# meuleman/epilogos

Hardware: AMD Instinct MI355X
Metric: Mbins scored/sec (S1, 18-state, 833 biosamples) (higher is better)
Workload: dtype u8

## Files before the change

### epilogos_amd/csrc/epg_s1.hip

```cpp
#include "epg_count.h"

#include <stdlib.h>
#include <string.h>

namespace epg {

typedef unsigned short k1_v2u16 __attribute__((ext_vector_type(2)));

constexpr int K1P_LD = 17;

template <int SC, bool FULL, bool PAIRS, typename Loop>
__device__ __forceinline__ void bin_hist_body(int Sout_, u64* __restrict__ counts, int nmax, u64* __restrict__ counts2, Loop&& loop) {
    constexpr int S = SC;
    constexpr int ND = (S + 1) / 2;
    const int Sout = FULL ? S : Sout_;
    const int ROWB = 2 * Sout;
    __shared__ u64 s_cnt[S + 1];
    __shared__ __attribute__((aligned(16))) char s_stage[4][32 * 2 * S];
    constexpr int PG = (S + 2) / 3, PSP = 3 * PG, PROLES = PG * (PG + 1) / 2, PSLICE = PROLES <= 64 ? 64 / PROLES : 1;
    static_assert(!PAIRS || (FULL && PROLES <= 64), "the pair counts need a compile-time row width and at most 64 block roles");
    __shared__ u32 s_pair[PAIRS ? 4 * PSP * K1P_LD : 1];
    __shared__ u64 s_c2[PAIRS ? S * S : 1];
    const int lane = threadIdx.x & 63, wave = threadIdx.x >> 6;
    const int j = lane & 3, b = lane >> 2;
    if (threadIdx.x <= S) s_cnt[threadIdx.x] = 0;
    if (PAIRS) {
        for (int e = threadIdx.x; e < S * S; e += 256) s_c2[e] = 0;
        for (int e = threadIdx.x; e < 4 * PSP * K1P_LD; e += 256) s_pair[e] = 0;
    }
    __syncthreads();
    u16* H = nullptr;
    int pgi = -1, pgj = 0, pkq = 0;
    u64 pacc[PAIRS ? 9 : 1], prs[PAIRS ? 3 : 1];
    if (PAIRS) {
        const int role = lane < PROLES * PSLICE ? lane / PSLICE : -1;
        pkq = lane % PSLICE;
        if (role >= 0) {
            int t = role, i = 0;
            while (t >= PG - i) { t -= PG - i; ++i; }
            pgi = i; pgj = i + t;
        }
#pragma unroll
        for (int c = 0; c < 9; ++c) pacc[c] = 0;
#pragma unroll
        for (int c = 0; c < 3; ++c) prs[c] = 0;
    }
    auto pair_counts = [&](const char* stage, int rows) {
        u32* sp = s_pair + wave * PSP * K1P_LD;
        const u16* raw = reinterpret_cast<const u16*>(stage);
        __builtin_amdgcn_wave_barrier();
        for (int e = lane; e < S * 16; e += 64) {
            const int i = e >> 4, k = e & 15;
            const u32 lo = 2 * k < rows ? raw[(2 * k) * S + i] : 0u, hi = 2 * k + 1 < rows ? raw[(2 * k + 1) * S + i] : 0u;
            sp[i * K1P_LD + k] = lo | (hi << 16);
        }
        __builtin_amdgcn_wave_barrier();
        if (pgi >= 0) {
            const u32* pi = sp + 3 * pgi * K1P_LD;
            const u32* pj = sp + 3 * pgj * K1P_LD;
            u32 part[9] = {0, 0, 0, 0, 0, 0, 0, 0, 0}, ps[3] = {0, 0, 0};
            const bool diag = pgi == pgj;
            for (int k = pkq; k < 16; k += PSLICE) {
                const u32 av[3] = {pi[k], pi[K1P_LD + k], pi[2 * K1P_LD + k]};
                const u32 bv[3] = {pj[k], pj[K1P_LD + k], pj[2 * K1P_LD + k]};
#pragma unroll
                for (int t = 0; t < 3; ++t)
#pragma unroll
                    for (int u = 0; u < 3; ++u)
                        part[3 * t + u] = __builtin_amdgcn_udot2(__builtin_bit_cast(k1_v2u16, av[t]), __builtin_bit_cast(k1_v2u16, bv[u]), part[3 * t + u], false);
                if (diag) {
#pragma unroll
                    for (int t = 0; t < 3; ++t)
                        ps[t] = __builtin_amdgcn_udot2(__builtin_bit_cast(k1_v2u16, av[t]), __builtin_bit_cast(k1_v2u16, 0x00010001u), ps[t], false);
                }
            }
#pragma unroll
            for (int c = 0; c < 9; ++c) pacc[c] += part[c];
#pragma unroll
            for (int c = 0; c < 3; ++c) prs[c] += ps[c];
        }
        __builtin_amdgcn_wave_barrier();
    };

    u32 accp[ND];
#pragma unroll
    for (int m = 0; m < ND; ++m) accp[m] = 0;
    const int flush_every = 65535 / nmax > 1 ? 65535 / nmax - 1 : 1;
    int since = 0;
    auto flush = [&]() {
        if (j == 0) {
#pragma unroll
            for (int m = 0; m < ND; ++m) {
                const u32 lo = accp[m] & 0xffffu, hi = accp[m] >> 16;
                if (lo) atomicAdd(&s_cnt[2 * m], (u64)lo);
                if (hi) atomicAdd(&s_cnt[2 * m + 1], (u64)hi);
            }
        }
#pragma unroll
        for (int m = 0; m < ND; ++m) accp[m] = 0;
        since = 0;
    };

    auto enter = [&](u16* Hpart) { H = Hpart; };
    auto epilogue = [&](int half, long row, bool valid, u32 (&cnt)[S]) {
        u32 d[ND];
        pack_reduce<S>(cnt, d);
        if (counts) {
#pragma unroll
            for (int m = 0; m < ND; ++m) accp[m] += valid ? d[m] : 0u;
            if (++since >= flush_every) flush();
        }
        if (H) {
            char* srow = &s_stage[wave][(half * 16 + b) * ROWB];
            if constexpr (FULL && (S & 1) == 0) {
#pragma unroll
                for (int k = 0; k < (ND + 3) / 4; ++k) {
                    const u32 v = sel4(d[4 * k], 4 * k + 1 < ND ? d[4 * k + 1] : 0u, 4 * k + 2 < ND ? d[4 * k + 2] : 0u,
                                       4 * k + 3 < ND ? d[4 * k + 3] : 0u, j);
                    if (4 * k + j < ND) *reinterpret_cast<u32*>(srow + 4 * (4 * k + j)) = v;
                }
            } else {
#pragma unroll
                for (int k = 0; k < (S + 3) / 4; ++k) {
                    const u32 v = (j & 2) ? (2 * k + 1 < ND ? d[2 * k + 1] : 0u) : d[2 * k];
                    const u32 c = (j & 1) ? v >> 16 : v & 0xffffu;
                    if (4 * k + j < Sout) *reinterpret_cast<u16*>(srow + 2 * (4 * k + j)) = (u16)c;
                }
            }
        }
    };
    auto finish = [&](long st, long row0, int rows) {
        if (H) store_staged(s_stage[wave], reinterpret_cast<char*>(H) + row0 * ROWB, rows * ROWB, lane);
        if constexpr (PAIRS) pair_counts(s_stage[wave], rows);
    };
    loop(enter, epilogue, finish);

    if (counts) {
        flush();
        __syncthreads();
        if ((int)threadIdx.x < Sout && s_cnt[threadIdx.x]) atomicAdd(&counts[threadIdx.x], s_cnt[threadIdx.x]);
    }
    if constexpr (PAIRS) {
        if (pgi >= 0) {
            const bool diag = pgi == pgj;
#pragma unroll
            for (int t = 0; t < 3; ++t)
#pragma unroll
                for (int u = 0; u < 3; ++u) {
                    const int i = 3 * pgi + t, jj = 3 * pgj + u;
                    u64 v = pacc[3 * t + u];
                    if (diag && t == u) v -= prs[t];
                    if (i >= S || jj >= S || !v) continue;
                    atomicAdd(&s_c2[i * S + jj], v);
                    if (!diag) atomicAdd(&s_c2[jj * S + i], v);
                }
        }
        __syncthreads();
        for (int e = threadIdx.x; e < S * S; e += 256)
            if (s_c2[e]) atomicAdd(&counts2[e], s_c2[e]);
    }
}

template <int SC, int NG, bool FULL>
__global__ __launch_bounds__(256) void k_bin_hist(const char* __restrict__ X, long R, int N, long ldx, int Sout_,
                                                   u16* __restrict__ H, u64* __restrict__ counts) {
    bin_hist_body<SC, FULL, false>(Sout_, counts, N, nullptr, [&](auto&& enter, auto&& epilogue, auto&& finish) {
        enter(H);
        tile_loop<SC, NG>(X, R, N, ldx, epilogue, finish);
    });
}

template <int SC, int NG>
__global__ __launch_bounds__(256) void k_bin_hist_s2(const char* __restrict__ X, long R, int N, long ldx, u16* __restrict__ H,
                                                      u64* __restrict__ counts, u64* __restrict__ counts2) {
    bin_hist_body<SC, true, true>(SC, counts, N, counts2, [&](auto&& enter, auto&& epilogue, auto&& finish) {
        enter(H);
        tile_loop<SC, NG>(X, R, N, ldx, epilogue, finish);
    });
}

template <int SC, int NG, bool FULL>
__global__ __launch_bounds__(256) void k_bin_hist_parts(const KhParts pt, int Sout_, u64* __restrict__ counts, int nmax) {
    bin_hist_body<SC, FULL, false>(Sout_, counts, nmax, nullptr, [&](auto&& enter, auto&& epilogue, auto&& finish) {
        tile_loop_parts<SC, NG>(pt, [&](int part) { enter(pt.h[part]); }, epilogue, finish);
    });
}

__global__ __launch_bounds__(256) void k_bin_hist_safe(const char* __restrict__ X, long row_begin, long row_end, int N,
                                                        long ldx, int S, u16* __restrict__ H, u64* __restrict__ counts, int mask = 31) {
    __shared__ u32 s_h[4][128];
    const int lane = threadIdx.x & 63, wave = threadIdx.x >> 6;
    for (long row = row_begin + (long)blockIdx.x * 4 + wave; row < row_end; row += (long)gridDim.x * 4) {
        for (int s = lane; s < S; s += 64) s_h[wave][s] = 0;
        __builtin_amdgcn_wave_barrier();
        const char* rp = X + row * ldx;
        for (int n = lane; n < N; n += 64) {
            const int v = (unsigned char)rp[n] & mask;
            if (v < S) atomicAdd(&s_h[wave][v], 1u);
        }
        __builtin_amdgcn_wave_barrier();
        for (int s = lane; s < S; s += 64) {
            const u32 c = s_h[wave][s];
            if (H) H[row * S + s] = (u16)c;
            if (counts && c) atomicAdd(&counts[s], (u64)c);
        }
        __builtin_amdgcn_wave_barrier();
    }
}

__global__ void k_s1_table(const float* __restrict__ q, int N, int S, double* __restrict__ T64, float* __restrict__ T32) {
    const long e = (long)blockIdx.x * blockDim.x + threadIdx.x;
    if (e >= (long)(N + 1) * S) return;
    const int c = (int)(e / S), s = (int)(e % S);
    const double p = (double)c / (double)N;
    const double v = kl_term(p, (double)q[s]);
    T64[e] = v;
    T32[e] = (float)v;
}

template <int S, int NG, typename OT>
__global__ __launch_bounds__(256) void k_score_s1(const char* __restrict__ X, long R, int N, long ldx,
                                                   const OT* __restrict__ T, OT* __restrict__ out) {
    constexpr int ND = (S + 1) / 2;
    constexpr int ROWB = S * (int)sizeof(OT);
    __shared__ __attribute__((aligned(16))) char s_stage[4][32 * ROWB];
    const int lane = threadIdx.x & 63, wave = threadIdx.x >> 6;
    const int j = lane & 3, b = lane >> 2;
    auto epilogue = [&](int half, long row, bool valid, u32 (&cnt)[S]) {
        u32 d[ND];
        pack_reduce<S>(cnt, d);
        OT* srow = reinterpret_cast<OT*>(&s_stage[wave][(half * 16 + b) * ROWB]);
#pragma unroll
        for (int k = 0; k < (S + 3) / 4; ++k) {
            const u32 v = (j & 2) ? (2 * k + 1 < ND ? d[2 * k + 1] : 0u) : d[2 * k];
            const u32 c = (j & 1) ? v >> 16 : v & 0xffffu;
            const int s = 4 * k + j;
            if (s < S) srow[s] = (c && valid) ? T[(long)c * S + s] : (OT)0;
        }
    };
    auto finish = [&](long st, long row0, int rows) {
        store_staged_nt(s_stage[wave], reinterpret_cast<char*>(out) + row0 * ROWB, rows * ROWB, lane);
    };
    tile_loop<S, NG>(X, R, N, ldx, epilogue, finish);
}

template <typename OT, bool LDS_T>
__global__ __launch_bounds__(LDS_T ? 1024 : 256) void k_score_s1_from_hist(const u16* __restrict__ H, long total, int S,
                                                                             const OT* __restrict__ Tg, int nent, OT* __restrict__ out,
                                                                             u64* __restrict__ zero_counts, int rev) {
    extern __shared__ __attribute__((aligned(16))) char smem_t[];
    if (zero_counts && blockIdx.x == 0 && (int)threadIdx.x < S) zero_counts[threadIdx.x] = 0;
    const OT* T = Tg;
    if (LDS_T) {
        OT* Ts = reinterpret_cast<OT*>(smem_t);
        for (int e = threadIdx.x; e < nent; e += blockDim.x) Ts[e] = Tg[e];
        __syncthreads();
        T = Ts;
    }
    const u32 cmax = (u32)(nent / S - 1);
    const long nquads = total >> 2;
    const long stride = (long)gridDim.x * blockDim.x;
    long qd = (long)blockIdx.x * blockDim.x + threadIdx.x;
    const long qtop = nquads - 1, qsgn = rev ? -1 : 1, qoff = rev ? qtop : 0;
    for (; qd + 3 * stride < nquads; qd += 4 * stride) {
        uint2 h[4];
#pragma unroll
        for (int u = 0; u < 4; ++u) h[u] = *reinterpret_cast<const uint2*>(H + 4 * (qoff + qsgn * (qd + u * stride)));
#pragma unroll
        for (int u = 0; u < 4; ++u) {
            const long e0 = 4 * (qoff + qsgn * (qd + u * stride));
            int s = (int)(e0 % S);
            const u32 c[4] = {h[u].x & 0xffffu, h[u].x >> 16, h[u].y & 0xffffu, h[u].y >> 16};
            OT v[4];
#pragma unroll
            for (int k = 0; k < 4; ++k) {
                v[k] = c[k] - 1u < cmax ? T[(long)c[k] * S + s] : (OT)0;
                s = s + 1 == S ? 0 : s + 1;
            }
            if constexpr (sizeof(OT) == 4) {
                typedef float v4f_nt __attribute__((ext_vector_type(4)));
                const v4f_nt vv = {(float)v[0], (float)v[1], (float)v[2], (float)v[3]};
                __builtin_nontemporal_store(vv, reinterpret_cast<v4f_nt*>(out + e0));
            } else {
                typedef double v2d_nt __attribute__((ext_vector_type(2)));
                const v2d_nt lo = {(double)v[0], (double)v[1]}, hi = {(double)v[2], (double)v[3]};
                __builtin_nontemporal_store(lo, reinterpret_cast<v2d_nt*>(out + e0));
                __builtin_nontemporal_store(hi, reinterpret_cast<v2d_nt*>(out + e0 + 2));
            }
        }
    }
    for (; qd < nquads; qd += stride) {
        const long e0 = 4 * (qoff + qsgn * qd);
        int s = (int)(e0 % S);
        for (int k = 0; k < 4; ++k) {
            const u32 c = H[e0 + k];
            out[e0 + k] = c - 1u < cmax ? T[(long)c * S + s] : (OT)0;
            s = s + 1 == S ? 0 : s + 1;
        }
    }
    if (blockIdx.x == 0 && threadIdx.x < (total & 3)) {
        const long e = (nquads << 2) + threadIdx.x;
        const u32 c = H[e];
        out[e] = c - 1u < cmax ? T[(long)c * S + (int)(e % S)] : (OT)0;
    }
}

template <typename IT>
__global__ __launch_bounds__(256) void k_sum_int(const IT* __restrict__ C, long n, long long* __restrict__ total) {
    long long acc = 0;
    for (long i = (long)blockIdx.x * blockDim.x + threadIdx.x; i < n; i += (long)gridDim.x * blockDim.x) acc += (long long)C[i];
    for (int off = 32; off > 0; off >>= 1) acc += __shfl_down(acc, off);
    __shared__ long long s_part[4];
    if ((threadIdx.x & 63) == 0) s_part[threadIdx.x >> 6] = acc;
    __syncthreads();
    if (threadIdx.x == 0) {
        const long long t = s_part[0] + s_part[1] + s_part[2] + s_part[3];
        if (t) atomicAdd(reinterpret_cast<u64*>(total), (u64)t);
    }
}

template <typename IT>
__global__ __launch_bounds__(256) void k_normalise(const IT* __restrict__ C, long n, const long long* __restrict__ total,
                                                    float* __restrict__ q) {
    const double tot = (double)(*total);
    for (long i = (long)blockIdx.x * blockDim.x + threadIdx.x; i < n; i += (long)gridDim.x * blockDim.x)
        q[i] = (float)((double)C[i] / tot);
}

template <typename IT>
__global__ __launch_bounds__(256) void k_normalise_small(const IT* __restrict__ C, int n, float* __restrict__ q) {
    __shared__ long long s_part[4];
    long long acc = 0;
    for (int i = threadIdx.x; i < n; i += 256) acc += (long long)C[i];
    for (int off = 32; off > 0; off >>= 1) acc += __shfl_down(acc, off);
    if ((threadIdx.x & 63) == 0) s_part[threadIdx.x >> 6] = acc;
    __syncthreads();
    const double tot = (double)(s_part[0] + s_part[1] + s_part[2] + s_part[3]);
    for (int i = threadIdx.x; i < n; i += 256) q[i] = (float)((double)C[i] / tot);
}

static int blocks_per_cu() { return g_force[FORCE_K1_BLOCKS_PER_CU] > 0 ? g_force[FORCE_K1_BLOCKS_PER_CU] : 2; }
static int grid_for_tiles(long R) {
    const long nsuper = (R + 31) >> 5;
    long blocks = (nsuper + 3) / 4;
    const long cap = (long)num_cus() * blocks_per_cu();
    if (blocks > cap) {
        const long iters = (nsuper + cap * 4 - 1) / (cap * 4);
        blocks = (nsuper + iters * 4 - 1) / (iters * 4);
    }
    if (blocks < 1) blocks = 1;
    return (int)blocks;
}

template <typename F>
static void with_count_core(int S, int ng, F&& f) {
    if (S == 15 || S == 18 || S == 25)
        with_constant<25, 15, 18>(S, [&](auto sc) {
            with_constant<0, 1, 2, 3, 4, 5, 6, 7, 8>(ng, [&](auto NG) { f(sc, NG, std::true_type{}); });
        });
    else
        with_constant<31, 15, 18, 25>(S < 15 ? 15 : S < 18 ? 18 : S < 25 ? 25 : 31,
                                      [&](auto sc) { f(sc, std::integral_constant<int, 0>{}, std::false_type{}); });
}

static long fast_rows(long R, int N, long ldx) {
    const long chunks = (N + 15) / 16;
    const long over = 16 * chunks - ldx;
    if (over <= 0) return R;
    const long unsafe = (over + ldx - 1) / ldx;
    return R > unsafe ? R - unsafe : 0;
}

extern "C" int epg_bin_hist(const int8_t* X8, int64_t R, int32_t N, int64_t ldx, int32_t S, uint16_t* H, int64_t* counts, void* stream) {
    hipStream_t st = (hipStream_t)stream;
    if (R < 0 || N < 1 || ldx < N || S < 1) return fail(EPG_ERR_INVALID_ARG, "bin_hist: bad shape R=%lld N=%d ldx=%lld S=%d", (long long)R, N, (long long)ldx, S);
    if (S > 127) return fail(EPG_ERR_UNSUPPORTED, "bin_hist: S=%d > 127 (states are int8)", S);
    if (N > 65535) return fail(EPG_ERR_UNSUPPORTED, "bin_hist: N=%d > 65535 (uint16 per-bin counts)", N);
    if (R == 0) return EPG_OK;
    if (!X8) return fail(EPG_ERR_INVALID_ARG, "bin_hist: X is NULL");
    if (H && (reinterpret_cast<uintptr_t>(H) & 15)) return fail(EPG_ERR_INVALID_ARG, "bin_hist: H must be 16-byte aligned");
    const char* X = reinterpret_cast<const char*>(X8);
    u64* cnt = reinterpret_cast<u64*>(counts);
    if (S > 31) {
        hipLaunchKernelGGL(k_bin_hist_safe, dim3((unsigned)((R + 3) / 4 < num_cus() * 32L ? (R + 3) / 4 : num_cus() * 32L)), dim3(256), 0, st, X, 0L,
                           (long)R, N, ldx, S, H, cnt, 255);
        EPG_LAUNCH_CHECK("k_bin_hist_safe");
        return EPG_OK;
    }
    const long Rf = fast_rows(R, N, ldx);
    if (Rf > 0) {
        with_count_core(S, (N + 127) / 128, [&](auto SC, auto NG, auto MODEL) {
            hipLaunchKernelGGL((k_bin_hist<SC, NG, MODEL && (SC & 1) == 0>), dim3(grid_for_tiles(Rf)), dim3(256), 0, st, X, Rf, N, ldx, S, H, cnt);
        });
        EPG_LAUNCH_CHECK("k_bin_hist");
    }
    if (Rf < R) {
        hipLaunchKernelGGL(k_bin_hist_safe, dim3((unsigned)((R - Rf + 3) / 4 < 1024 ? (R - Rf + 3) / 4 : 1024)), dim3(256), 0, st, X, Rf, (long)R, N, ldx, S, H, cnt);
        EPG_LAUNCH_CHECK("k_bin_hist_safe");
    }
    return EPG_OK;
}

extern "C" int epg_bin_hist_s2(const int8_t* X8, int64_t R, int32_t N, int64_t ldx, int32_t S, uint16_t* H, int64_t* counts, int64_t* counts2,
                               void* stream) {
    hipStream_t st = (hipStream_t)stream;
    if (!H || !counts2) return fail(EPG_ERR_INVALID_ARG, "bin_hist_s2: H and counts2 are required");
    const bool fused = (S == 15 || S == 18 || S == 25) && R > 0 && N >= 1 && N <= 1024 && ldx >= N && X8 &&
                       !(reinterpret_cast<uintptr_t>(H) & 15) && fast_rows(R, N, ldx) == R;
    if (!fused) {
        int rc = epg_bin_hist(X8, R, N, ldx, S, H, counts, stream);
        if (rc) return rc;
        return epg_hist_s2_from_binhist(H, R, S, counts2, stream);
    }
    const char* X = reinterpret_cast<const char*>(X8);
    u64* c1 = reinterpret_cast<u64*>(counts);
    u64* c2 = reinterpret_cast<u64*>(counts2);
    with_constant<25, 18, 15>(S, [&](auto SC) {
        with_constant<8, 1, 2, 3, 4, 5, 6, 7>((N + 127) / 128, [&](auto NG) {
            hipLaunchKernelGGL((k_bin_hist_s2<decltype(SC)::value, NG>), dim3(grid_for_tiles(R)), dim3(256), 0, st, X, R, N, ldx, H, c1, c2);
        });
    });
    EPG_LAUNCH_CHECK("k_bin_hist_s2");
    return EPG_OK;
}

extern "C" int epg_bin_hist_parts(int32_t nparts, const int8_t* const* X, const int64_t* R, const int32_t* N, const int64_t* ldx, int32_t S,
                                  uint16_t* const* H, int64_t* counts, void* stream) {
    hipStream_t st = (hipStream_t)stream;
    if (nparts < 0 || (nparts && (!X || !R || !N || !ldx))) return fail(EPG_ERR_INVALID_ARG, "bin_hist_parts: NULL argument array");
    if (S < 1 || S > 127) return fail(EPG_ERR_UNSUPPORTED, "bin_hist_parts: S=%d outside 1..127", S);
    for (int p = 0; p < nparts; ++p) {
        if (R[p] < 0 || (R[p] && (N[p] < 1 || ldx[p] < N[p]))) return fail(EPG_ERR_INVALID_ARG, "bin_hist_parts: bad shape of part %d", p);
        if (R[p] && N[p] > 65535) return fail(EPG_ERR_UNSUPPORTED, "bin_hist_parts: N=%d > 65535 (uint16 per-bin counts)", N[p]);
        if (R[p] && !X[p]) return fail(EPG_ERR_INVALID_ARG, "bin_hist_parts: X of part %d is NULL", p);
        if (H && H[p] && (reinterpret_cast<uintptr_t>(H[p]) & 15)) return fail(EPG_ERR_INVALID_ARG, "bin_hist_parts: H of part %d must be 16-byte aligned", p);
    }
    if (S > 31) {
        for (int p = 0; p < nparts; ++p) {
            const int rc = epg_bin_hist(X[p], R[p], N[p], ldx[p], S, H ? H[p] : nullptr, counts, stream);
            if (rc) return rc;
        }
        return EPG_OK;
    }
    u64* cnt = reinterpret_cast<u64*>(counts);
    auto cls = [](int n) { const int ng = (n + 127) / 128; return ng <= 8 ? ng : 0; };
    bool seen[9] = {false, false, false, false, false, false, false, false, false};
    for (int p = 0; p < nparts; ++p)
        if (R[p]) seen[cls(N[p])] = true;
    for (int c = 0; c <= 8; ++c) {
        if (!seen[c]) continue;
        for (int p0 = 0; p0 < nparts;) {
            KhParts pt;
            memset(&pt, 0, sizeof(pt));
            long supers = 0;
            int nmax = 1, p = p0;
            for (; p < nparts && pt.n < KH_MAXP; ++p) {
                if (!R[p] || cls(N[p]) != c) continue;
                const long Rf = fast_rows(R[p], N[p], ldx[p]);
                if (Rf < R[p]) {
                    hipLaunchKernelGGL(k_bin_hist_safe, dim3((unsigned)((R[p] - Rf + 3) / 4 < 1024 ? (R[p] - Rf + 3) / 4 : 1024)), dim3(256), 0, st,
                                       reinterpret_cast<const char*>(X[p]), Rf, (long)R[p], N[p], (long)ldx[p], S, H ? H[p] : nullptr, cnt);
                    EPG_LAUNCH_CHECK("k_bin_hist_safe");
                }
                if (Rf == 0) continue;
                const int k = pt.n++;
                pt.x[k] = reinterpret_cast<const char*>(X[p]);
                pt.h[k] = H ? H[p] : nullptr;
                pt.rows[k] = Rf;
                pt.ldx[k] = ldx[p];
                pt.n_cols[k] = N[p];
                pt.st0[k] = supers;
                supers += (Rf + 31) / 32;
                if (N[p] > nmax) nmax = N[p];
            }
            pt.st0[pt.n] = supers;
            p0 = p;
            if (pt.n == 0) break;
            with_count_core(S, c, [&](auto SC, auto NG, auto) {
                hipLaunchKernelGGL((k_bin_hist_parts<SC, NG, (NG > 0 && (SC & 1) == 0)>), dim3(grid_for_tiles(supers * 32)), dim3(256), 0, st, pt, S,
                                   cnt, nmax);
            });
            EPG_LAUNCH_CHECK("k_bin_hist_parts");
        }
    }
    return EPG_OK;
}

static int64_t s1_table_bytes(int N, int S) { return align_up((int64_t)(N + 1) * S * 8, 256) + align_up((int64_t)(N + 1) * S * 4, 256); }

int64_t s1_ws_bytes(int64_t R, int N, int S) {
    return s1_table_bytes(N, S) + 256 + align_up(R * S * 2, 256);
}

static int build_s1_table(const float* q, int N, int S, void* ws, double** T64, float** T32, hipStream_t st) {
    *T64 = reinterpret_cast<double*>(ws);
    *T32 = reinterpret_cast<float*>(reinterpret_cast<char*>(ws) + align_up((int64_t)(N + 1) * S * 8, 256));
    const long n = (long)(N + 1) * S;
    hipLaunchKernelGGL(k_s1_table, dim3((int)((n + 255) / 256)), dim3(256), 0, st, q, N, S, *T64, *T32);
    EPG_LAUNCH_CHECK("k_s1_table");
    return EPG_OK;
}
static int check_score_from_hist_args(const uint16_t* H, const double* out64, const float* out32) {
    if ((reinterpret_cast<uintptr_t>(H) & 7) != 0) return fail(EPG_ERR_INVALID_ARG, "score_s1_from_binhist: H must be 8-byte aligned");
    if ((out32 && (reinterpret_cast<uintptr_t>(out32) & 15)) || (out64 && (reinterpret_cast<uintptr_t>(out64) & 15)))
        return fail(EPG_ERR_INVALID_ARG, "score_s1_from_binhist: outputs must be 16-byte aligned");
    return EPG_OK;
}

template <typename OT>
static int launch_score_s1_from_hist_t(const uint16_t* H, long total, int32_t S, const OT* T, int nent, OT* out, u64* zero_counts, hipStream_t st) {
    const size_t tbytes = (size_t)nent * sizeof(OT);
    const int rev = 1;
    if (tbytes <= 150 * 1024) {
        const int per_cu = tbytes <= 75 * 1024 ? 2 : 1;
        long nb = (total / 4 + 4095) / 4096;
        if (nb > (long)num_cus() * per_cu) nb = (long)num_cus() * per_cu;
        if (nb < 1) nb = 1;
        auto kern = k_score_s1_from_hist<OT, true>;
        static DynLds lds_attr;
        EPG_HIP(ensure_dyn_lds(lds_attr, reinterpret_cast<const void*>(kern), 150 * 1024));
        hipLaunchKernelGGL(kern, dim3((int)nb), dim3(1024), tbytes, st, H, total, S, T, nent, out, zero_counts, rev);
    } else {
        long nb = (total / 4 + 1023) / 1024;
        if (nb > num_cus() * 8L) nb = num_cus() * 8L;
        if (nb < 1) nb = 1;
        hipLaunchKernelGGL((k_score_s1_from_hist<OT, false>), dim3((int)nb), dim3(256), 0, st, H, total, S, T, nent, out, zero_counts, rev);
    }
    EPG_LAUNCH_CHECK("k_score_s1_from_hist");
    return EPG_OK;
}

static int launch_score_s1_from_hist(const uint16_t* H, int64_t R, int32_t N, int32_t S, const double* T64, const float* T32,
                                     double* out64, float* out32, hipStream_t st, u64* zero_counts = nullptr) {
    const long total = (long)R * S;
    const int nent = (N + 1) * S;
    int rc = EPG_OK;
    if (out32) rc = launch_score_s1_from_hist_t<float>(H, total, S, T32, nent, out32, zero_counts, st);
    if (!rc && out64) rc = launch_score_s1_from_hist_t<double>(H, total, S, T64, nent, out64, out32 ? nullptr : zero_counts, st);
    return rc;
}


extern "C" int epg_score_s1_from_binhist(const uint16_t* H, int64_t R, int32_t N, int32_t S, const float* q, double* out64, float* out32,
                                         void* ws, int64_t ws_bytes, void* stream) {
    hipStream_t st = (hipStream_t)stream;
    if (R < 0 || N < 1 || S < 1) return fail(EPG_ERR_INVALID_ARG, "score_s1: bad shape");
    if (R == 0) return EPG_OK;
    if (!H || !q || !ws) return fail(EPG_ERR_INVALID_ARG, "score_s1_from_binhist: NULL argument");
    if (ws_bytes < s1_table_bytes(N, S)) return fail(EPG_ERR_WORKSPACE, "score_s1: workspace %lld < %lld bytes", (long long)ws_bytes, (long long)s1_table_bytes(N, S));
    int rc = check_score_from_hist_args(H, out64, out32);
    if (rc) return rc;
    double* T64; float* T32;
    rc = build_s1_table(q, N, S, ws, &T64, &T32, st);
    if (rc) return rc;
    return launch_score_s1_from_hist(H, R, N, S, T64, T32, out64, out32, st);
}

extern "C" int epg_score_s1_from_binhist_table(const uint16_t* H, int64_t R, int32_t N, int32_t S, const double* T64, const float* T32,
                                               double* out64, float* out32, void* stream) {
    if (R < 0 || N < 1 || S < 1) return fail(EPG_ERR_INVALID_ARG, "score_s1: bad shape");
    if (R == 0) return EPG_OK;
    if (!H || (out64 && !T64) || (out32 && !T32)) return fail(EPG_ERR_INVALID_ARG, "score_s1_from_binhist_table: NULL argument");
    if ((T64 && (reinterpret_cast<uintptr_t>(T64) & 7)) || (T32 && (reinterpret_cast<uintptr_t>(T32) & 3)))
        return fail(EPG_ERR_INVALID_ARG, "score_s1_from_binhist_table: misaligned table");
    int rc = check_score_from_hist_args(H, out64, out32);
    if (rc) return rc;
    return launch_score_s1_from_hist(H, R, N, S, T64, T32, out64, out32, (hipStream_t)stream);
}

__global__ __launch_bounds__(256) void k_s1_combine(const u64* __restrict__ counts, int N, int S, float* __restrict__ q,
                                                     double* __restrict__ T64, float* __restrict__ T32) {
    __shared__ long long s_c[128];
    __shared__ double s_q[128];
    const int t = threadIdx.x;
    if (t < S) s_c[t] = (long long)counts[t];
    __syncthreads();
    if (t < S) {
        long long tot = 0;
        for (int s = 0; s < S; ++s) tot += s_c[s];
        const float qf = (float)((double)s_c[t] / (double)tot);
        if (blockIdx.x == 0) q[t] = qf;
        s_q[t] = (double)qf;
    }
    __syncthreads();
    const int e = blockIdx.x * 256 + t;
    if (e < (N + 1) * S) {
        const int c = e / S, s = e - c * S;
        const double v = kl_term((double)c / (double)N, s_q[s]);
        T64[e] = v;
        T32[e] = (float)v;
    }
}

extern "C" int epg_combine_score_s1(int64_t* counts, int32_t rezero, const uint16_t* H, int64_t R, int32_t N, int32_t S, float* q,
                                    double* out64, float* out32, void* ws, int64_t ws_bytes, void* stream) {
    hipStream_t st = (hipStream_t)stream;
    if (R < 0 || N < 1 || S < 1) return fail(EPG_ERR_INVALID_ARG, "combine_score_s1: bad shape R=%lld N=%d S=%d", (long long)R, N, S);
    if (S > 127) return fail(EPG_ERR_UNSUPPORTED, "combine_score_s1: S=%d > 127 (states are int8)", S);
    if (!counts || !q || !ws || (R > 0 && !H)) return fail(EPG_ERR_INVALID_ARG, "combine_score_s1: NULL argument");
    if (ws_bytes < s1_table_bytes(N, S)) return fail(EPG_ERR_WORKSPACE, "combine_score_s1: workspace %lld < %lld bytes", (long long)ws_bytes, (long long)s1_table_bytes(N, S));
    int rc = check_score_from_hist_args(H, out64, out32);
    if (rc) return rc;
    double* T64 = reinterpret_cast<double*>(ws);
    float* T32 = reinterpret_cast<float*>(reinterpret_cast<char*>(ws) + align_up((int64_t)(N + 1) * S * 8, 256));
    const long nent = (long)(N + 1) * S;
    hipLaunchKernelGGL(k_s1_combine, dim3((unsigned)((nent + 255) / 256)), dim3(256), 0, st, reinterpret_cast<const u64*>(counts), N, S, q, T64, T32);
    EPG_LAUNCH_CHECK("k_s1_combine");
    if (R == 0 || (!out32 && !out64)) {
        if (rezero) EPG_HIP(hipMemsetAsync(counts, 0, (size_t)S * 8, st));
        return EPG_OK;
    }
    return launch_score_s1_from_hist(H, R, N, S, T64, T32, out64, out32, st, rezero ? reinterpret_cast<u64*>(counts) : nullptr);
}

extern "C" int epg_hist_s1(const int8_t* X, int64_t R, int32_t N, int64_t ldx, int32_t S, int64_t* counts, void* stream) {
    if (!counts) return fail(EPG_ERR_INVALID_ARG, "hist_s1: counts is NULL");
    return epg_bin_hist(X, R, N, ldx, S, nullptr, counts, stream);
}

extern "C" int epg_score_s1(const int8_t* X8, int64_t R, int32_t N, int64_t ldx, int32_t S, const float* q, double* out64, float* out32,
                            void* ws, int64_t ws_bytes, void* stream) {
    hipStream_t st = (hipStream_t)stream;
    if (R < 0 || N < 1 || ldx < N || S < 1) return fail(EPG_ERR_INVALID_ARG, "score_s1: bad shape");
    if (S > 127) return fail(EPG_ERR_UNSUPPORTED, "score_s1: S=%d > 127 (states are int8)", S);
    if (R == 0) return EPG_OK;
    if (!X8 || !q || !ws) return fail(EPG_ERR_INVALID_ARG, "score_s1: NULL argument");
    if ((out32 && (reinterpret_cast<uintptr_t>(out32) & 15)) || (out64 && (reinterpret_cast<uintptr_t>(out64) & 15)))
        return fail(EPG_ERR_INVALID_ARG, "score_s1: outputs must be 16-byte aligned");
    const long Rf = fast_rows(R, N, ldx);
    const bool fused = S == 18 && Rf == R;
    if (!fused) {
        if (ws_bytes < s1_ws_bytes(R, N, S)) return fail(EPG_ERR_WORKSPACE, "score_s1: workspace %lld < %lld bytes", (long long)ws_bytes, (long long)s1_ws_bytes(R, N, S));
        u16* H = reinterpret_cast<u16*>(reinterpret_cast<char*>(ws) + s1_table_bytes(N, S));
        int rc = epg_bin_hist(X8, R, N, ldx, S, H, nullptr, stream);
        if (rc) return rc;
        return epg_score_s1_from_binhist(H, R, N, S, q, out64, out32, ws, s1_table_bytes(N, S), stream);
    }
    if (ws_bytes < s1_table_bytes(N, S)) return fail(EPG_ERR_WORKSPACE, "score_s1: workspace %lld < %lld bytes", (long long)ws_bytes, (long long)s1_table_bytes(N, S));
    double* T64; float* T32;
    int rc = build_s1_table(q, N, S, ws, &T64, &T32, st);
    if (rc) return rc;
    const char* X = reinterpret_cast<const char*>(X8);
    with_constant<0, 1, 2, 3, 4, 5, 6, 7, 8>((N + 127) / 128, [&](auto NG) {
        if (out32) hipLaunchKernelGGL((k_score_s1<18, NG, float>), dim3(grid_for_tiles(R)), dim3(256), 0, st, X, R, N, ldx, T32, out32);
        if (out64) hipLaunchKernelGGL((k_score_s1<18, NG, double>), dim3(grid_for_tiles(R)), dim3(256), 0, st, X, R, N, ldx, T64, out64);
    });
    EPG_LAUNCH_CHECK("k_score_s1");
    return EPG_OK;
}

template <typename IT>
static int normalise_impl(const IT* C, int64_t n, float* q, void* ws, int64_t ws_bytes, hipStream_t st) {
    if (n < 1 || !C || !q || !ws) return fail(EPG_ERR_INVALID_ARG, "normalise: bad argument");
    if (ws_bytes < 8) return fail(EPG_ERR_WORKSPACE, "normalise: workspace needs 8 bytes");
    if (n <= 4096) {
        hipLaunchKernelGGL((k_normalise_small<IT>), dim3(1), dim3(256), 0, st, C, (int)n, q);
        EPG_LAUNCH_CHECK("k_normalise_small");
        return EPG_OK;
    }
    long long* total = reinterpret_cast<long long*>(ws);
    EPG_HIP(hipMemsetAsync(total, 0, 8, st));
    long blocks = (n + 255) / 256;
    if (blocks > num_cus() * 8L) blocks = num_cus() * 8L;
    hipLaunchKernelGGL((k_sum_int<IT>), dim3((int)blocks), dim3(256), 0, st, C, (long)n, total);
    hipLaunchKernelGGL((k_normalise<IT>), dim3((int)blocks), dim3(256), 0, st, C, (long)n, total, q);
    EPG_LAUNCH_CHECK("k_normalise");
    return EPG_OK;
}

extern "C" int epg_normalise_i64(const int64_t* C, int64_t n, float* q, void* ws, int64_t ws_bytes, void* stream) {
    return normalise_impl<long long>(reinterpret_cast<const long long*>(C), n, q, ws, ws_bytes, (hipStream_t)stream);
}
extern "C" int epg_normalise_i32(const int32_t* C, int64_t n, float* q, void* ws, int64_t ws_bytes, void* stream) {
    return normalise_impl<int>(C, n, q, ws, ws_bytes, (hipStream_t)stream);
}

}
```

Before: 5795.

## Rewrite S1 score-from-histogram kernel as wave-tiled streaming with branchless LDS lookup

Replaces the quad-per-thread score kernel with a per-wave 512-element tiled streaming kernel. It uses 16-byte histogram loads, software-prefetched double buffering and a padded LDS table, where row 0 and a sentinel row are zeroed so lookups are branchless. State offsets are tracked incrementally, with the grid sized so each tile's state phase advances by a fixed step instead of a modulo per element. For f32, a DPP lane swap lets each lane write contiguous 16-byte nontemporal stores, and the state count is specialized at compile time. The aim is to cut per-element index arithmetic and branching and to improve load and store vector width, at the cost of considerably more complex tail and alignment handling.

New measurement: 5827 (median of 4 runs). About the same (+0.6%).

```diff
diff --git a/epilogos_amd/csrc/epg_s1.hip b/epilogos_amd/csrc/epg_s1.hip
--- a/epilogos_amd/csrc/epg_s1.hip
+++ b/epilogos_amd/csrc/epg_s1.hip
@@ -244,64 +244,153 @@
     tile_loop<S, NG>(X, R, N, ldx, epilogue, finish);
 }
 
-template <typename OT, bool LDS_T>
-__global__ __launch_bounds__(LDS_T ? 1024 : 256) void k_score_s1_from_hist(const u16* __restrict__ H, long total, int S,
-                                                                             const OT* __restrict__ Tg, int nent, OT* __restrict__ out,
-                                                                             u64* __restrict__ zero_counts, int rev) {
+constexpr int SS_TILE = 512;
+constexpr int SS_STORE_F32 = 1, SS_STORE_F64 = 0, SS_THREADS = 1024, SS_UNROLL = 2;
+typedef float ss_f32x4 __attribute__((ext_vector_type(4)));
+typedef double ss_f64x2 __attribute__((ext_vector_type(2)));
+
+template <typename OT>
+__device__ __forceinline__ void ss_store4_nt(OT* p, OT a, OT b, OT c, OT d) {
+    if constexpr (sizeof(OT) == 4) {
+        const ss_f32x4 v = {a, b, c, d};
+        __builtin_nontemporal_store(v, reinterpret_cast<ss_f32x4*>(p));
+    } else {
+        const ss_f64x2 lo = {a, b}, hi = {c, d};
+        __builtin_nontemporal_store(lo, reinterpret_cast<ss_f64x2*>(p));
+        __builtin_nontemporal_store(hi, reinterpret_cast<ss_f64x2*>(p + 2));
+    }
+}
+
+template <typename OT, int SC, bool LDS_T, int STORE, int NT, int U>
+__global__ __launch_bounds__(NT) void k_score_s1_stream(const u16* __restrict__ H, long total, int S_, int N, const OT* __restrict__ Tg,
+                                                         OT* __restrict__ out, u64* __restrict__ zero_counts, int rev, int step) {
     extern __shared__ __attribute__((aligned(16))) char smem_t[];
-    if (zero_counts && blockIdx.x == 0 && (int)threadIdx.x < S) zero_counts[threadIdx.x] = 0;
-    const OT* T = Tg;
+    constexpr int SZ = (int)sizeof(OT), WPB = NT / 64;
+    static_assert(STORE != 1 || SZ == 4, "the pair swap is laid out for 4-byte scores");
+    const int S = SC ? SC : S_;
+    const int tid = threadIdx.x, lane = tid & 63, wave = tid >> 6;
+    if (zero_counts && blockIdx.x == 0 && tid < S) zero_counts[tid] = 0;
+    const long head = (reinterpret_cast<uintptr_t>(H) & 8) ? (total < 4 ? total : 4) : 0;
+    const long ntiles = (total - head) / SS_TILE;
+    const long GW = (long)gridDim.x * WPB;
+    long t = (long)blockIdx.x * WPB + wave;
+    auto tile_elem = [&](long tt) { return head + (rev ? ntiles - 1 - tt : tt) * SS_TILE; };
+    const int lunit = STORE == 1 ? (lane >> 1) + 32 * (lane & 1) : lane;
+    const int o0 = STORE == 1 ? 4 * lane : 8 * lane, o1 = STORE == 1 ? 256 + 4 * lane : 8 * lane + 4;
+    auto load_tile = [&](long tt) { return *reinterpret_cast<const uint4*>(H + tile_elem(tt) + 8 * lunit); };
+    uint4 h[U];
+    bool have = t + (U - 1) * GW < ntiles;
+    if (have) {
+#pragma unroll
+        for (int u = 0; u < U; ++u) h[u] = load_tile(t + u * GW);
+    }
+    const u32 rowb = (u32)(S * SZ);
+    const u32 stage_off = LDS_T ? (u32)(((N + 2) * S * SZ + 15) & ~15) : 0u;
     if (LDS_T) {
         OT* Ts = reinterpret_cast<OT*>(smem_t);
-        for (int e = threadIdx.x; e < nent; e += blockDim.x) Ts[e] = Tg[e];
+        const int nent = (N + 1) * S;
+        constexpr int V = 16 / SZ;
+        typedef OT ss_vec __attribute__((ext_vector_type(V)));
+        const int nv = (reinterpret_cast<uintptr_t>(Tg) & 15) ? 0 : nent / V;
+        for (int i = tid; i < nv; i += NT) {
+            ss_vec v = reinterpret_cast<const ss_vec*>(Tg)[i];
+#pragma unroll
+            for (int j = 0; j < V; ++j)
+                if (i * V + j < S) v[j] = (OT)0;
+            reinterpret_cast<ss_vec*>(Ts)[i] = v;
+        }
+        for (int e = nv * V + tid; e < nent; e += NT) Ts[e] = e < S ? (OT)0 : Tg[e];
+        for (int e = nent + tid; e < nent + S; e += NT) Ts[e] = (OT)0;
         __syncthreads();
-        T = Ts;
-    }
-    const u32 cmax = (u32)(nent / S - 1);
-    const long nquads = total >> 2;
-    const long stride = (long)gridDim.x * blockDim.x;
-    long qd = (long)blockIdx.x * blockDim.x + threadIdx.x;
-    const long qtop = nquads - 1, qsgn = rev ? -1 : 1, qoff = rev ? qtop : 0;
-    for (; qd + 3 * stride < nquads; qd += 4 * stride) {
-        uint2 h[4];
-#pragma unroll
-        for (int u = 0; u < 4; ++u) h[u] = *reinterpret_cast<const uint2*>(H + 4 * (qoff + qsgn * (qd + u * stride)));
-#pragma unroll
-        for (int u = 0; u < 4; ++u) {
-            const long e0 = 4 * (qoff + qsgn * (qd + u * stride));
-            int s = (int)(e0 % S);
-            const u32 c[4] = {h[u].x & 0xffffu, h[u].x >> 16, h[u].y & 0xffffu, h[u].y >> 16};
-            OT v[4];
+    }
+    auto lookup = [&](u32 c, u32 soff) -> OT {
+        if constexpr (LDS_T) {
+            c = min(c, (u32)N + 1u);
+            return *reinterpret_cast<const OT*>(smem_t + (c * rowb + soff));
+        } else {
+            const OT x = *reinterpret_cast<const OT*>(reinterpret_cast<const char*>(Tg) + (min(c, (u32)N) * rowb + soff));
+            return c - 1u < (u32)N ? x : (OT)0;
+        }
+    };
+    u32 sb[8];
+    const int o0m = o0 % S, o1m = o1 % S;
+    auto set_bases = [&](int st) {
+#pragma unroll
+        for (int j = 0; j < 2; ++j) {
+            int s = st + (j ? o1m : o0m);
+            s -= s >= S ? S : 0;
 #pragma unroll
             for (int k = 0; k < 4; ++k) {
-                v[k] = c[k] - 1u < cmax ? T[(long)c[k] * S + s] : (OT)0;
+                sb[4 * j + k] = (u32)(s * SZ);
                 s = s + 1 == S ? 0 : s + 1;
             }
-            if constexpr (sizeof(OT) == 4) {
-                typedef float v4f_nt __attribute__((ext_vector_type(4)));
-                const v4f_nt vv = {(float)v[0], (float)v[1], (float)v[2], (float)v[3]};
-                __builtin_nontemporal_store(vv, reinterpret_cast<v4f_nt*>(out + e0));
-            } else {
-                typedef double v2d_nt __attribute__((ext_vector_type(2)));
-                const v2d_nt lo = {(double)v[0], (double)v[1]}, hi = {(double)v[2], (double)v[3]};
-                __builtin_nontemporal_store(lo, reinterpret_cast<v2d_nt*>(out + e0));
-                __builtin_nontemporal_store(hi, reinterpret_cast<v2d_nt*>(out + e0 + 2));
-            }
-        }
-    }
-    for (; qd < nquads; qd += stride) {
-        const long e0 = 4 * (qoff + qsgn * qd);
-        int s = (int)(e0 % S);
-        for (int k = 0; k < 4; ++k) {
-            const u32 c = H[e0 + k];
-            out[e0 + k] = c - 1u < cmax ? T[(long)c * S + s] : (OT)0;
-            s = s + 1 == S ? 0 : s + 1;
-        }
-    }
-    if (blockIdx.x == 0 && threadIdx.x < (total & 3)) {
-        const long e = (nquads << 2) + threadIdx.x;
-        const u32 c = H[e];
-        out[e] = c - 1u < cmax ? T[(long)c * S + (int)(e % S)] : (OT)0;
+        }
+    };
+    int st = t < ntiles ? (int)((u64)tile_elem(t) % (u32)S) : 0;
+    const int stepv = rev && step ? S - step : step;
+    set_bases(st);
+    auto process = [&](const uint4& hv, long tt) {
+        u32 w[4] = {hv.x, hv.y, hv.z, hv.w};
+        if constexpr (STORE == 1) {
+            const bool odd = lane & 1;
+            const u32 a = (u32)__builtin_amdgcn_update_dpp(0, (int)(odd ? w[0] : w[2]), 0xB1, 0xf, 0xf, false);
+            const u32 b = (u32)__builtin_amdgcn_update_dpp(0, (int)(odd ? w[1] : w[3]), 0xB1, 0xf, 0xf, false);
+            w[0] = odd ? a : w[0]; w[1] = odd ? b : w[1];
+            w[2] = odd ? w[2] : a; w[3] = odd ? w[3] : b;
+        }
+        OT v[8];
+#pragma unroll
+        for (int i = 0; i < 8; ++i) v[i] = lookup((i & 1) ? w[i >> 1] >> 16 : w[i >> 1] & 0xffffu, sb[i]);
+        OT* o = out + tile_elem(tt);
+        if constexpr (STORE == 2) {
+            char* stg = smem_t + stage_off + wave * (SS_TILE * SZ);
+            typedef u32 ss_u32x4 __attribute__((ext_vector_type(4)));
+            __builtin_amdgcn_fence(__ATOMIC_RELEASE, "workgroup");
+            __builtin_amdgcn_wave_barrier();
+            OT* mine = reinterpret_cast<OT*>(stg) + 8 * lane;
+#pragma unroll
+            for (int i = 0; i < 8; ++i) mine[i] = v[i];
+            __builtin_amdgcn_fence(__ATOMIC_RELEASE, "workgroup");
+            __builtin_amdgcn_wave_barrier();
+            __builtin_amdgcn_fence(__ATOMIC_ACQUIRE, "workgroup");
+#pragma unroll
+            for (int k = 0; k < SZ / 2; ++k)
+                __builtin_nontemporal_store(*reinterpret_cast<const ss_u32x4*>(stg + 16 * (64 * k + lane)),
+                                            reinterpret_cast<ss_u32x4*>(reinterpret_cast<char*>(o) + 16 * (64 * k + lane)));
+        } else {
+            ss_store4_nt(o + o0, v[0], v[1], v[2], v[3]);
+            ss_store4_nt(o + o1, v[4], v[5], v[6], v[7]);
+        }
+        if (step) {
+            st += stepv;
+            st -= st >= S ? S : 0;
+            set_bases(st);
+        }
+    };
+    while (have) {
+        const long tn = t + U * GW;
+        const bool haven = tn + (U - 1) * GW < ntiles;
+        uint4 hn[U];
+#pragma unroll
+        for (int u = 0; u < U; ++u) hn[u] = h[u];
+        if (haven) {
+#pragma unroll
+            for (int u = 0; u < U; ++u) hn[u] = load_tile(tn + u * GW);
+        }
+#pragma unroll
+        for (int u = 0; u < U; ++u) process(h[u], t + u * GW);
+#pragma unroll
+        for (int u = 0; u < U; ++u) h[u] = hn[u];
+        t = tn;
+        have = haven;
+    }
+    for (; t < ntiles; t += GW) process(load_tile(t), t);
+    if (blockIdx.x == gridDim.x - 1) {
+        const long tail0 = head + ntiles * SS_TILE, nrest = head + (total - tail0);
+        for (long i = tid; i < nrest; i += NT) {
+            const long e = i < head ? i : tail0 + (i - head);
+            out[e] = lookup(H[e], (u32)((int)(e % S) * SZ));
+        }
     }
 }
 
@@ -507,36 +596,65 @@
     return EPG_OK;
 }
 
+static long ss_gcd(long a, long b) { return b ? ss_gcd(b, a % b) : a; }
+
+template <typename OT, int SC, bool LDS_T, int STORE, int NT, int U>
+static int launch_score_s1_stream(const uint16_t* H, long total, int32_t S, int32_t N, const OT* T, OT* out, u64* zero_counts, int per_cu,
+                                  hipStream_t st) {
+    constexpr int SZ = (int)sizeof(OT), WPB = NT / 64;
+    const size_t lds = (LDS_T ? (size_t)align_up((int64_t)(N + 2) * S * SZ, 16) : 0) + (STORE == 2 ? (size_t)WPB * SS_TILE * SZ : 0);
+    if (lds > 160 * 1024) return fail(EPG_ERR_UNSUPPORTED, "score_s1_from_binhist: %zu bytes of LDS", lds);
+    if (LDS_T && 2 * lds > 160 * 1024) per_cu = 1;
+    const int rev = 1;
+    const long cap = (long)num_cus() * per_cu;
+    long nb = (total / SS_TILE + WPB - 1) / WPB;
+    if (nb >= cap) {
+        nb = cap;
+        const long m = S / ss_gcd(S, (long)SS_TILE * WPB);
+        if (nb >= m) nb -= nb % m;
+    }
+    if (nb < 1) nb = 1;
+    const int step = (int)(((long)SS_TILE * WPB * nb) % S);
+    auto kern = k_score_s1_stream<OT, SC, LDS_T, STORE, NT, U>;
+    if (lds > 48 * 1024) {
+        static DynLds lds_attr;
+        EPG_HIP(ensure_dyn_lds(lds_attr, reinterpret_cast<const void*>(kern), 160 * 1024));
+    }
+    hipLaunchKernelGGL(kern, dim3((unsigned)nb), dim3(NT), lds, st, H, total, S, N, T, out, zero_counts, rev, step);
+    EPG_LAUNCH_CHECK("k_score_s1_stream");
+    return EPG_OK;
+}
+
 template <typename OT>
-static int launch_score_s1_from_hist_t(const uint16_t* H, long total, int32_t S, const OT* T, int nent, OT* out, u64* zero_counts, hipStream_t st) {
-    const size_t tbytes = (size_t)nent * sizeof(OT);
-    const int rev = 1;
-    if (tbytes <= 150 * 1024) {
-        const int per_cu = tbytes <= 75 * 1024 ? 2 : 1;
-        long nb = (total / 4 + 4095) / 4096;
-        if (nb > (long)num_cus() * per_cu) nb = (long)num_cus() * per_cu;
-        if (nb < 1) nb = 1;
-        auto kern = k_score_s1_from_hist<OT, true>;
-        static DynLds lds_attr;
-        EPG_HIP(ensure_dyn_lds(lds_attr, reinterpret_cast<const void*>(kern), 150 * 1024));
-        hipLaunchKernelGGL(kern, dim3((int)nb), dim3(1024), tbytes, st, H, total, S, T, nent, out, zero_counts, rev);
-    } else {
-        long nb = (total / 4 + 1023) / 1024;
-        if (nb > num_cus() * 8L) nb = num_cus() * 8L;
-        if (nb < 1) nb = 1;
-        hipLaunchKernelGGL((k_score_s1_from_hist<OT, false>), dim3((int)nb), dim3(256), 0, st, H, total, S, T, nent, out, zero_counts, rev);
-    }
-    EPG_LAUNCH_CHECK("k_score_s1_from_hist");
-    return EPG_OK;
+static int launch_score_s1_from_hist_t(const uint16_t* H, long total, int32_t S, int32_t N, const OT* T, OT* out, u64* zero_counts, hipStream_t st) {
+    const bool lds_t = (size_t)(N + 1) * S * sizeof(OT) <= 150 * 1024;
+    constexpr int STORE = sizeof(OT) == 4 ? SS_STORE_F32 : SS_STORE_F64;
+#ifdef EPILOGOS_BUILD_EXPERIMENTS
+    if (const char* e = exp_env("EPG_S1S"); e && S == 18 && lds_t) {
+        int sto = 0, nt = 1024, un = 2, pc = 2;
+        sscanf(e, "%d,%d,%d,%d", &sto, &nt, &un, &pc);
+        if (sizeof(OT) == 8 && sto == 1) sto = 0;
+#define SS_TRY(STO, NT_, U_) \
+        if (sto == STO && nt == NT_ && un == U_) return launch_score_s1_stream<OT, 18, true, (sizeof(OT) == 8 && STO == 1) ? 0 : STO, NT_, U_>(H, total, S, N, T, out, zero_counts, pc, st);
+#define SS_TRY_U(STO, NT_) SS_TRY(STO, NT_, 1) SS_TRY(STO, NT_, 2) SS_TRY(STO, NT_, 4)
+#define SS_TRY_NT(STO) SS_TRY_U(STO, 1024) SS_TRY_U(STO, 512) SS_TRY_U(STO, 256)
+        SS_TRY_NT(0) SS_TRY_NT(1) SS_TRY_NT(2)
+        return fail(EPG_ERR_INVALID_ARG, "EPG_S1S=%s: no such instantiation", e);
+    }
+#endif
+    return with_constant<0, 15, 18, 25>(S, [&](auto sc) {
+        constexpr int SC = decltype(sc)::value;
+        if (lds_t) return launch_score_s1_stream<OT, SC, true, STORE, SS_THREADS, SS_UNROLL>(H, total, S, N, T, out, zero_counts, 2, st);
+        return launch_score_s1_stream<OT, SC, false, sizeof(OT) == 4 ? 1 : 0, 256, 2>(H, total, S, N, T, out, zero_counts, 8, st);
+    });
 }
 
 static int launch_score_s1_from_hist(const uint16_t* H, int64_t R, int32_t N, int32_t S, const double* T64, const float* T32,
                                      double* out64, float* out32, hipStream_t st, u64* zero_counts = nullptr) {
     const long total = (long)R * S;
-    const int nent = (N + 1) * S;
     int rc = EPG_OK;
-    if (out32) rc = launch_score_s1_from_hist_t<float>(H, total, S, T32, nent, out32, zero_counts, st);
-    if (!rc && out64) rc = launch_score_s1_from_hist_t<double>(H, total, S, T64, nent, out64, out32 ? nullptr : zero_counts, st);
+    if (out32) rc = launch_score_s1_from_hist_t<float>(H, total, S, N, T32, out32, zero_counts, st);
+    if (!rc && out64) rc = launch_score_s1_from_hist_t<double>(H, total, S, N, T64, out64, out32 ? nullptr : zero_counts, st);
     return rc;
 }
 
```
